# nanoporetech/pomfret

Hardware: AMD Instinct MI355X
Metric: aligned reads/sec (methphase kernel) (higher is better)
Workload: dtype u32/f32

## Files before the change

### pomfret_amd/csrc/pf_kernels.hip

```cpp
#include <hip/hip_runtime.h>
#include <stdint.h>
#include "pf_device.h"

#define DEV static __device__ __forceinline__

#ifdef PF_K3_PROFILE
DEV unsigned long long k3_stamp_now() {
    unsigned long long t;
    __builtin_amdgcn_sched_barrier(0);
    asm volatile("s_memtime %0\n\ts_waitcnt lgkmcnt(0)" : "=s"(t) :: "memory");
    __builtin_amdgcn_sched_barrier(0);
    return t;
}
#define K3_STAMP(i) do { const unsigned long long t_ = k3_stamp_now(); \
    prof_acc[i] += t_ - prof_last; prof_last = t_; } while (0)
DEV unsigned long long k3_realtime() {
    unsigned long long t;
    asm volatile("s_memrealtime %0\n\ts_waitcnt lgkmcnt(0)" : "=s"(t) :: "memory");
    return t;
}
#define K3_COUNT(i, v) do { prof_acc[i] += (v); } while (0)
#define K12_STAMP(i) do { if (threadIdx.x == 0) { const unsigned long long t_ = k3_stamp_now(); \
    d.prof[64ull * d.W + (uint64_t)w * 16 + (i)] = t_ - k12_t0; k12_t0 = t_; } } while (0)
#define K2_STAMP(i) do { if (k2acc) { const unsigned long long t_ = k3_stamp_now(); \
    k2acc[i] += t_ - k2acc[9]; k2acc[9] = t_; } } while (0)
#else
#define K12_STAMP(i) do { } while (0)
#define K2_STAMP(i) do { } while (0)
#define K3_STAMP(i) do { } while (0)
#define K3_COUNT(i, v) do { } while (0)
#endif

#ifdef PF_ASM_MARK
#define K3_MARK(s) asm volatile("; MARK " s)
#else
#define K3_MARK(s) do { } while (0)
#endif

DEV uint32_t uni(uint32_t x) { return (uint32_t)__builtin_amdgcn_readfirstlane((int)x); }
DEV int uni_i(int x) { return __builtin_amdgcn_readfirstlane(x); }

DEV uint64_t lanemask_lt(uint32_t lane) { return lane ? (~0ull >> (64 - lane)) : 0ull; }

DEV void wave_sync() {
    __builtin_amdgcn_fence(__ATOMIC_RELEASE, "wavefront");
    __builtin_amdgcn_wave_barrier();
    __builtin_amdgcn_fence(__ATOMIC_ACQUIRE, "wavefront");
}

DEV void wave_sync_mem() {
    __builtin_amdgcn_fence(__ATOMIC_RELEASE, "workgroup");
    __builtin_amdgcn_wave_barrier();
    __builtin_amdgcn_fence(__ATOMIC_ACQUIRE, "workgroup");
}

DEV uint32_t wave_incl_scan(uint32_t x, uint32_t lane) {
#pragma unroll
    for (int o = 1; o < 64; o <<= 1) {
        uint32_t y = __shfl_up(x, o, 64);
        if (lane >= (uint32_t)o) x += y;
    }
    return x;
}

DEV uint32_t wave_max_u32(uint32_t x) {
#pragma unroll
    for (int o = 32; o > 0; o >>= 1) { uint32_t y = __shfl_xor(x, o, 64); x = y > x ? y : x; }
    return x;
}

DEV uint32_t dpp_max_step(uint32_t x, const int ctrl_sel) {
    uint32_t y;
    switch (ctrl_sel) {
    case 0: y = (uint32_t)__builtin_amdgcn_update_dpp(0, (int)x, 0xB1, 0xF, 0xF, false); break;
    case 1: y = (uint32_t)__builtin_amdgcn_update_dpp(0, (int)x, 0x4E, 0xF, 0xF, false); break;
    case 2: y = (uint32_t)__builtin_amdgcn_update_dpp(0, (int)x, 0x141, 0xF, 0xF, false); break;
    default: y = (uint32_t)__builtin_amdgcn_update_dpp(0, (int)x, 0x140, 0xF, 0xF, false); break;
    }
    return y > x ? y : x;
}
DEV uint32_t wave_max_dpp(uint32_t x) {
    x = dpp_max_step(x, 0);
    x = dpp_max_step(x, 1);
    x = dpp_max_step(x, 2);
    x = dpp_max_step(x, 3);
    const uint32_t a = (uint32_t)__builtin_amdgcn_readlane((int)x, 0), b = (uint32_t)__builtin_amdgcn_readlane((int)x, 16);
    const uint32_t c = (uint32_t)__builtin_amdgcn_readlane((int)x, 32), e = (uint32_t)__builtin_amdgcn_readlane((int)x, 48);
    const uint32_t ab = a > b ? a : b, ce = c > e ? c : e;
    return ab > ce ? ab : ce;
}
DEV uint32_t wave_shl1(uint32_t x) {
    return (uint32_t)__builtin_amdgcn_update_dpp(0, (int)x, 0x130, 0xF, 0xF, false);
}
DEV float div_u16_y(float fa, float fb, float y) {
    const float q0 = fa * y;
    const float r = __builtin_fmaf(-q0, fb, fa);
    return __builtin_fmaf(r, y, q0);
}
DEV float div_u16(uint32_t a, uint32_t b) {
    const float fb = (float)b;
    return div_u16_y((float)a, fb, __builtin_amdgcn_rcpf(fb));
}
DEV float4 site_rec(uint32_t v) {
    const uint32_t h0 = v & 0xffffu, h1 = v >> 16;
    const float f0 = (float)(h0 ? h0 : 1u), f1 = (float)(h1 ? h1 : 1u);
    return make_float4(f0, f1, h0 ? __builtin_amdgcn_rcpf(f0) : 0.f, h1 ? __builtin_amdgcn_rcpf(f1) : 0.f);
}

DEV uint32_t dpp_shr_add(uint32_t x, const int ctrl) {
    uint32_t y;
    switch (ctrl) {
    case 1: y = (uint32_t)__builtin_amdgcn_update_dpp(0, (int)x, 0x111, 0xF, 0xF, true); break;
    case 2: y = (uint32_t)__builtin_amdgcn_update_dpp(0, (int)x, 0x112, 0xF, 0xF, true); break;
// ... 1225 lines not shown
            const uint32_t r = r0 + i;
            d.mmr_off[2 * r] = kcarry + 2ull * e1;
            d.mmr_off[2 * r + 1] = kcarry + 2ull * e1 + bound;
            d.big_off[r] = bigb ? bcarry + e2 : ~0ull;
        }
        kcarry += 2ull * t1;
        bcarry += t2;
    }

    K12_STAMP(5);
    const uint32_t arr_b = (uint32_t)((14ull * S + 15) & ~15ull);
    if (tid == 0) sh_misc[5] = NW;
    __syncthreads();

    if (staged && R >= d.k12c_minr && S <= d.k12c_smax) {
        for (uint32_t c = tid; c * PF_K12C_READS < R; c += NT) {
            const uint32_t k = atomicAdd(d.k12c_ctr, 1u);
            d.k12c_list[2ull * k] = w;
            d.k12c_list[2ull * k + 1] = c * PF_K12C_READS;
        }
    } else if (staged) {
        uint8_t *wb = reinterpret_cast<uint8_t *>(tile) + arr_b + wid * (uint64_t)PF_K12_WB * PF_K12_CAPW;
#ifdef PF_K3_PROFILE
        unsigned long long k2a[10] = {0, 0, 0, 0, 0, 0, 0, 0, 0, __builtin_amdgcn_s_memtime()};
        unsigned long long *k2acc = wid == 0 ? k2a : nullptr;
#else
        unsigned long long *k2acc = nullptr;
#endif
        k12_methmers(d, r0, 0, R, wid, NW, lane, S, sp, st1, q1s, l0s, l1s, wb, k2acc, &sh_misc[5]);
#ifdef PF_K3_PROFILE
        if (tid == 0) {
            for (int j = 0; j < 7; j++) d.prof[64ull * d.W + (uint64_t)w * 16 + 8 + j] = k2a[j];
            d.prof[64ull * d.W + (uint64_t)w * 16 + 7] = k2a[7];
            d.prof[64ull * d.W + (uint64_t)w * 16 + 15] = k2a[8];
        }
#endif
    } else {
        for (uint32_t i = tid; i < R; i += NT) d.fb_list[atomicAdd(d.fb_ctr, 1u)] = r0 + i;
    }
    __syncthreads();
    K12_STAMP(6);
}

__global__ __launch_bounds__(PF_K12C_WAVES * 64) __attribute__((amdgpu_waves_per_eu(4, 4))) void pf_k12_chunks(pf_dev_batch d) {
    extern __shared__ __attribute__((aligned(16))) uint8_t smem[];
    __shared__ uint32_t s_item, s_rctr;
    const uint32_t tid = threadIdx.x, lane = tid & 63u, wid = uni(tid >> 6);
    const uint32_t n = *d.k12c_ctr;
    for (;;) {
        if (tid == 0) s_item = atomicAdd(d.k12c_next, 1u);
        __syncthreads();
        const uint32_t it = s_item;
        if (it >= n) break;
        const uint32_t w = d.k12c_list[2ull * it], c0 = d.k12c_list[2ull * it + 1];
        if (tid == 0) s_rctr = c0 + PF_K12C_WAVES;
        const uint32_t r0 = d.win_read_off[w], R = d.win_read_off[w + 1] - r0;
        const uint32_t S = d.win_S[w];
        const uint64_t sb = d.win_site_off[w];
        uint32_t *sp = reinterpret_cast<uint32_t *>(smem), *st1 = sp + S, *q1s = sp + 2 * S;
        uint8_t *l0s = reinterpret_cast<uint8_t *>(sp + 3 * S), *l1s = l0s + S;
        for (uint32_t p = tid; p < S; p += PF_K12C_WAVES * 64) {
            sp[p] = d.site_pos[sb + p];
            st1[p] = d.st1_pos[sb + p];
            q1s[p] = d.site_q1[sb + p];
            l0s[p] = d.len0[sb + p];
            l1s[p] = d.len1[sb + p];
        }
        __syncthreads();
        const uint32_t arr_b = (uint32_t)((14ull * S + 15) & ~15ull);
        uint8_t *wb = smem + arr_b + wid * (uint64_t)PF_K12_WB * PF_K12_CAPW;
        const uint32_t c1 = min(R, c0 + PF_K12C_READS);
        k12_methmers(d, r0, c0, c1, wid, PF_K12C_WAVES, lane, S, sp, st1, q1s, l0s, l1s, wb, nullptr,
                     &s_rctr);
        __syncthreads();
    }
}

struct K3Ctl {
    uint32_t S, R, ntot, nc, L, done, failed, inserted, winner, tag;
    int32_t i_last;
    uint32_t min_i, max_i, fail, summ, nstrict, mxlen, cmax;
    uint32_t path, need, cacheb;
    unsigned long long t_run;
    uint32_t ins_n, ins_st, ins_mo, ins_tg;
    unsigned long long scr;
    int32_t tab[4];
};

struct K3Cand {
    uint32_t read[PF_MAX_NCAND];
    uint32_t pos[PF_MAX_NCAND];
    uint32_t site0[PF_MAX_NCAND];
    uint32_t len[PF_MAX_NCAND];
    uint32_t kofs[PF_MAX_NCAND];
    unsigned long long key[PF_MAX_NCAND];
    uint8_t tag[PF_MAX_NCAND];
};

template <int NTH>
struct K3CandSlimT {
    uint32_t read[NTH];
    uint32_t pos[128];
    unsigned long long key[256];
};
using K3CandSlim = K3CandSlimT<PF_K3S_THREADS>;

DEV uint64_t align16(uint64_t x) { return (x + 15) & ~15ull; }

template <int NT, typename K, typename F>
DEV void k3_each_key(const pf_dev_batch &d, uint32_t r0, uint32_t R, uint32_t dir, K &&keep, F &&f) {
    constexpr uint32_t B = 8, NW = NT / 64;
    const uint32_t lane = threadIdx.x & 63, wid = threadIdx.x >> 6;
    for (uint32_t i0 = wid * B; i0 < R; i0 += NW * B) {
        uint32_t n[B], st[B], key[B];
        uint64_t off[B];
#pragma unroll
        for (uint32_t u = 0; u < B; u++) {
            const uint32_t i = i0 + u;
            const bool ok = i < R && keep(i);
            const uint64_t g = 2ull * (r0 + (ok ? i : 0u)) + dir;
            n[u] = ok ? d.mmr_n[g] : 0u;
            st[u] = d.mmr_start[g];
            off[u] = d.mmr_off[g];
        }
#pragma unroll
        for (uint32_t u = 0; u < B; u++) key[u] = lane < n[u] ? d.keys[off[u] + lane] : 0u;
#pragma unroll
        for (uint32_t u = 0; u < B; u++)
            if (lane < n[u]) f(i0 + u, lane, st[u] + lane, off[u] + lane, key[u]);
#pragma unroll
        for (uint32_t u = 0; u < B; u++)
            for (uint32_t t = 64 + lane; t < n[u]; t += 64) f(i0 + u, t, st[u] + t, off[u] + t, d.keys[off[u] + t]);
    }
}

template <int NT = PF_K3_THREADS>
DEV void k3_dict(const pf_dev_batch &d, uint32_t r0, uint32_t R, uint32_t S, uint32_t dir,
                 uint64_t *masks, uint32_t *base, uint32_t *sh_scan, K3Ctl &ctl) {
    const uint32_t tid = threadIdx.x;
    const uint32_t MW = (uint32_t)d.mw;
    for (uint32_t j = tid; j < S * MW; j += NT) masks[j] = 0;
    __syncthreads();
    k3_each_key<NT>(d, r0, R, dir, [](uint32_t) { return true; },
                    [&](uint32_t, uint32_t, uint32_t site, uint64_t, uint32_t key) {
                        if (site < S && key < 64u * MW)
                            atomicOr((unsigned long long *)&masks[(uint64_t)site * MW + (key >> 6)], 1ull << (key & 63));
                    });
    __syncthreads();
    uint32_t carry = 0;
    for (uint32_t p0 = 0; p0 < S; p0 += NT) {
        const uint32_t p = p0 + tid;
        uint32_t c = 0;
        if (p < S)
            for (uint32_t m = 0; m < MW; m++) c += (uint32_t)__popcll(masks[(uint64_t)p * MW + m]);
        uint32_t tot;
        const uint32_t ex = block_excl_scan<NT>(c, sh_scan, &tot);
        if (p < S) base[p] = carry + ex;
        carry += tot;
    }
    if (tid == 0) ctl.ntot = carry;
    __syncthreads();
}

template <int NT = PF_K3_THREADS>
DEV void k3_dict_rewrite(const pf_dev_batch &d, uint32_t r0, uint32_t R, uint32_t S, uint32_t dir,
                         const uint64_t *masks, const uint32_t *base) {
    const uint32_t MW = (uint32_t)d.mw;
    k3_each_key<NT>(d, r0, R, dir, [](uint32_t) { return true; },
                    [&](uint32_t, uint32_t, uint32_t site, uint64_t koff, uint32_t key) {
                        uint32_t slot = PF_NONE;
                        if (site < S && key < 64u * MW) {
                            const uint64_t *row = masks + (uint64_t)site * MW;
                            const uint32_t wi = key >> 6, b = key & 63;
                            slot = base[site];
                            for (uint32_t m = 0; m < wi; m++) slot += (uint32_t)__popcll(row[m]);
                            slot += (uint32_t)__popcll(row[wi] & ((1ull << b) - 1ull));
                        }
                        d.keys[koff] = slot;
                    });
    __syncthreads();
}

DEV uint32_t kd_hash(uint32_t key) {
    const uint32_t h = key * 0x9E3779B1u;
    return h ^ (h >> 15);
}
DEV void kd_sync() {
    __builtin_amdgcn_fence(__ATOMIC_RELEASE, "agent");
    __syncthreads();
    __builtin_amdgcn_fence(__ATOMIC_ACQUIRE, "agent");
}

__global__ __launch_bounds__(PF_K3_THREADS) void pf_k3_kdict(pf_dev_batch d) {
    constexpr uint32_t NT = PF_K3_THREADS, NW = NT / 64;
    __shared__ uint32_t sh_scan[NW + 1];
    __shared__ unsigned long long s_o;
    __shared__ uint32_t s_fail;
    const uint32_t prob = blockIdx.x, w = prob >> 1, dir = prob & 1;
    const uint32_t tid = threadIdx.x, lane = tid & 63u, wid = tid >> 6;
    const uint32_t S = d.win_S[w];
    if (S == 0) {
        if (tid == 0) d.k3_ntot[prob] = 0;
        return;
    }
    const uint32_t R = d.win_nreads[w], r0 = d.win_read_off[w];
    auto alloc = [&](uint64_t bytes) -> bool {
        if (tid == 0) {
            const unsigned long long o = atomicAdd(d.scr_ctr, (unsigned long long)bytes);
            s_fail = o + bytes > d.scr_cap;
            if (s_fail) atomicOr(d.status, PF_ST_SCR_OVF);
            s_o = o;
        }
        __syncthreads();
        return s_fail == 0;
    };
    if (!alloc(align16(12ull * (S + 1)))) { if (tid == 0) d.k3_ntot[prob] = PF_NONE; return; }
    uint32_t *cap = reinterpret_cast<uint32_t *>(d.scr + s_o), *toff = cap + (S + 1), *base = toff + (S + 1);
    for (uint32_t j = tid; j <= S; j += NT) cap[j] = 0;
    kd_sync();
    for (uint32_t i = tid; i < R; i += NT) {
        const uint64_t g = 2ull * (r0 + i) + dir;
        const uint32_t n = d.mmr_n[g], st = d.mmr_start[g];
        if (n && st < S) {
            atomicAdd(&cap[st], 1u);
            atomicAdd(&cap[st + n < S ? st + n : S], 0xFFFFFFFFu);
        }
    }
    kd_sync();
    const uint32_t per = (S + NT - 1) / NT, j0 = min(tid * per, S), j1 = min(j0 + per, S);
    uint32_t part = 0, tot = 0;
    for (uint32_t j = j0; j < j1; j++) part += cap[j];
// ... 590 lines not shown
template <bool SLDS, int NT = PF_K3_THREADS, bool C8 = false>
DEV void k3_init(const pf_dev_batch &d, uint32_t w, uint32_t dir, uint32_t r0, uint32_t S, uint32_t R,
                 const K3Mem &m, K3Ctl &ctl, uint32_t *sh_scan, K3Stats &stx) {
    const uint32_t tid = threadIdx.x, lane = tid & 63, wid = uni(tid >> 6);
    const uint32_t ntot = uni(ctl.ntot);
    const int cov_rt = d.win_par[w * 4 + 1];
    const uint32_t s = d.win_start[w], e = d.win_end[w];
    const uint32_t nwords = (R + 63) >> 6;
    const uint64_t sb = d.win_site_off[w];
    const uint64_t kbase = d.mmr_off[2ull * r0];
    const uint32_t *kb = d.keys + kbase;
    uint32_t sum_mmr = 0, mx_mmr = 0;
    for (uint32_t j = tid; j < (C8 ? (ntot + 1) / 2 : ntot); j += NT) m.cnt[j] = 0;
    for (uint32_t j = tid; j < S; j += NT) m.sum[j] = 0;
    for (uint32_t i = tid; i < R; i += NT) {
        const uint32_t r = r0 + i;
        const uint32_t st = d.read_start[r], en = d.read_end[r];
        uint32_t f = 0;
        if (st <= s) {
            f |= FLG_LEFT;
            if (en > s) f |= FLG_LEFT_STRICT;
        } else if (en >= e) {
            f |= FLG_RIGHT;
            if (st < e) f |= FLG_RIGHT_STRICT;
        }
        m.flg[i] = (uint8_t)f;
        m.hp[i] = d.read_hp[r];
        m.aux[i] = 0;
        if (dir) m.ord[i] = (uint16_t)d.rev_ord[r];
        const uint64_t g = 2ull * r + dir;
        const uint32_t n_ = d.mmr_n[g], st_ = d.mmr_start[g];
        if (!m.mn) {
        } else if (m.m16) {
            static_cast<uint16_t *>(m.mn)[i] = (uint16_t)n_;
            static_cast<uint16_t *>(m.mst)[i] = (uint16_t)st_;
        } else {
            static_cast<uint32_t *>(m.mn)[i] = n_;
            static_cast<uint32_t *>(m.mst)[i] = st_;
        }
        sum_mmr += n_;
        mx_mmr = n_ > mx_mmr ? n_ : mx_mmr;
    }
    if (tid == 0) {
        const uint32_t *a = d.site_pos + sb;
        if (dir == 0) {
            ctl.min_i = 0;
            ctl.max_i = (uint32_t)ub_u32(a, 0, S, s);
        } else {
            ctl.max_i = S - 1;
            ctl.min_i = (uint32_t)((int)ub_u32(a, 0, S, e) - 1);
        }
        ctl.i_last = dir == 0 ? 0 : (int)R - 1;
        ctl.failed = 0;
        ctl.done = 0;
        ctl.tab[0] = 0;
    }
    __syncthreads();
    if (SLDS) {
        uint32_t carry = 0;
        for (uint32_t i0 = 0; i0 < R; i0 += NT) {
            const uint32_t i = i0 + tid;
            const uint32_t v = i < R ? k3_mn(m, i) : 0;
            uint32_t tot;
            const uint32_t ex = block_excl_scan<NT>(v, sh_scan, &tot);
            if (i < R) m.mo[i] = carry + ex;
            carry += tot;
        }
        __syncthreads();
        for (uint32_t i = wid; i < R; i += (NT / 64)) {
            const uint32_t g = 2 * (r0 + i) + dir;
            const uint32_t *src = kb + (d.mmr_off[g] - kbase);
            uint16_t *dst = m.sl16 + m.mo[i];
            const uint32_t n = k3_mn(m, i);
            for (uint32_t t = lane; t < n; t += 64) {
                const uint32_t v = src[t];
                dst[t] = v == PF_NONE ? (uint16_t)0xFFFFu : (uint16_t)v;
            }
        }
    } else if (m.mo) {
        for (uint32_t i = tid; i < R; i += NT)
            m.mo[i] = (uint32_t)(d.mmr_off[2ull * (r0 + i) + dir] - kbase);
    }
    __syncthreads();
    const uint32_t refbit = dir == 0 ? FLG_LEFT : FLG_RIGHT;
    uint32_t ref_ins = 0;
    auto seed = [&](uint32_t i, uint32_t site, uint32_t slot) {
        const uint32_t hp = m.hp[i];
        if (site < S && slot != PF_NONE) {
            if (C8) atomicAdd(&m.cnt[slot >> 1], (hp ? 0x100u : 1u) << ((slot & 1u) * 16u));
            else atomicAdd(&m.cnt[slot], hp ? 0x10000u : 1u);
            atomicAdd(&m.sum[site], hp ? 0x10000u : 1u);
        }
    };
    auto is_ref = [&](uint32_t i) { return (m.flg[i] & refbit) && m.hp[i] <= 1; };
    if (SLDS) {
        for (uint32_t i = wid; i < R; i += (NT / 64)) {
            if (!is_ref(i)) continue;
            const uint32_t n = k3_mn(m, i), st = k3_mst(m, i), mo = m.mo[i];
            ref_ins += n;
            for (uint32_t t = lane; t < n; t += 64) seed(i, st + t, k3_slot<SLDS>(m, mo + t));
        }
    } else {
        k3_each_key<NT>(d, r0, R, dir, is_ref, [&](uint32_t i, uint32_t t, uint32_t site, uint64_t, uint32_t slot) {
            if (t == 0) ref_ins += d.mmr_n[2ull * (r0 + i) + dir];
            seed(i, site, slot);
        });
        ref_ins = (uint32_t)__builtin_amdgcn_readfirstlane((int)ref_ins);
    }
    if (lane == 0 && ref_ins) atomicAdd((uint32_t *)&ctl.tab[0], ref_ins);
    if (sum_mmr) atomicAdd(&ctl.summ, sum_mmr);
    if (mx_mmr) atomicMax(&ctl.mxlen, mx_mmr);
    __syncthreads();
    if (wid == 0) k3_range_update(m.sum, S, cov_rt, ctl, lane);
    for (uint32_t i = tid; i < R; i += NT) {
        if (m.flg[i] & refbit) {
            const uint32_t t = i | ((uint32_t)m.hp[i] >> 2);
            if (t < R) atomicMax(&m.aux[t], i + 1);
        }
    }
    __syncthreads();
    for (uint32_t i = tid; i < R; i += NT) {
        const uint32_t lw = m.aux[i];
        m.hp[i] = lw ? (uint8_t)(d.read_hp[r0 + lw - 1] & 3) : (uint8_t)2;
    }
    __syncthreads();
    for (uint32_t j = wid; j < nwords; j += (NT / 64)) {
        const uint32_t p = j * 64 + lane;
        bool u = false;
        if (p < R) {
            const uint32_t rd = dir ? m.ord[p] : p;
            const uint32_t h = m.hp[rd];
            u = h != 0 && h != 1;
        }
        const uint64_t b = __ballot(u);
        if (lane == 0) m.untag[j] = b;
    }
    stx.inserts = ctl.tab[0];
    __syncthreads();
}

DEV void k3_finish(const pf_dev_batch &d, uint32_t w, uint32_t dir, uint32_t r0, uint32_t S, uint32_t R,
                   const K3Mem &m, const K3Ctl &ctl, const K3Stats &stx) {
    const uint32_t lane = threadIdx.x & 63;
    int tab0 = 0, tab1 = 0, tab2 = 0, tab3 = 0;
    uint32_t nstrict = 0;
    const uint32_t strict = dir == 0 ? FLG_RIGHT_STRICT : FLG_LEFT_STRICT;
    for (uint32_t i = lane; i < R; i += 64) {
        if (m.flg[i] & strict) {
            nstrict++;
            const uint32_t ref = d.read_hp[r0 + i], q = m.hp[i];
            if (ref <= 1 && q <= 1) {
                const uint32_t k = ref * 2 + q;
                tab0 += k == 0; tab1 += k == 1; tab2 += k == 2; tab3 += k == 3;
            }
        }
        if (dir == 0) d.hp_fwd[r0 + i] = m.hp[i];
    }
    uint32_t tsum[5] = {(uint32_t)tab0, (uint32_t)tab1, (uint32_t)tab2, (uint32_t)tab3, nstrict};
#pragma unroll
    for (int k = 0; k < 5; k++) {
        uint32_t tot = 0;
        for (int bb = 0; bb < 16; bb++) tot += (uint32_t)__popcll(__ballot((tsum[k] >> bb) & 1)) << bb;
        tsum[k] = tot;
    }
    if (lane < 4) d.table[((uint64_t)w * 2 + dir) * 4 + lane] = (int32_t)tsum[lane];
    if (lane == 0) {
        unsigned long long *sp = d.stats + ((uint64_t)w * 2 + dir) * PF_NSTAT;
        sp[0] = stx.lookups; sp[1] = stx.inserts; sp[3] = stx.scanned;
        sp[2] = stx.iters | ((unsigned long long)ctl.path << 56);
        sp[4] = ctl.summ; sp[5] = tsum[4]; sp[6] = R; sp[7] = S;
    }
}


DEV void k3_range_regs(const K3Mem &m, uint32_t S, int cov_rt, uint32_t lane, uint32_t &umin, uint32_t &umax) {
    auto cov_ok = [&](int ii) -> bool {
        const uint32_t v = m.sum[ii];
        return (int)((v & 0xffffu) + (v >> 16)) >= cov_rt;
    };
    const int m0 = (int)umin, M0 = (int)umax;
    const bool left = lane < 32;
    const int i = left ? m0 - (int)lane : M0 + (int)(lane - 32);
    bool cvg = false;
    if (left ? (m0 >= 0 && i >= 0) : (M0 >= 0 && i < (int)S)) cvg = cov_ok(i);
    const uint64_t b = __ballot(cvg);
    const uint32_t bl = (uint32_t)b, br = (uint32_t)(b >> 32);
    int cl = bl == ~0u ? 32 : __ffs(~bl) - 1;
    int cr = br == ~0u ? 32 : __ffs(~br) - 1;
    if (cl == 32) {
        for (;;) {
            const int ii = m0 - cl - (int)lane;
            const uint64_t b2 = __ballot(ii >= 0 && cov_ok(ii));
            if (b2 == ~0ull) { cl += 64; continue; }
            cl += __ffsll((unsigned long long)~b2) - 1;
            break;
        }
    }
    if (cr == 32) {
        for (;;) {
            const int ii = M0 + cr + (int)lane;
            const uint64_t b2 = __ballot(ii < (int)S && cov_ok(ii));
            if (b2 == ~0ull) { cr += 64; continue; }
            cr += __ffsll((unsigned long long)~b2) - 1;
            break;
        }
    }
    if (m0 >= 0 && cl > 0) umin = (uint32_t)(m0 - cl + 1);
    if (M0 >= 0 && cr > 0) umax = (uint32_t)(M0 + cr - 1);
}

template <bool SLDS, int NT = PF_K3_THREADS, bool C8 = false, bool CACHE = false, typename CD = K3Cand>
DEV void k3_greedy_slim(const pf_dev_batch &d, uint32_t w, uint32_t dir, uint32_t r0, uint32_t S, uint32_t R,
                        const K3Mem &m, K3Ctl &ctl, CD &cd, uint32_t *sh_scan, uint32_t *qb, uint32_t CL = 0) {
    const uint32_t tid = threadIdx.x, lane = tid & 63, wid = uni(tid >> 6);
    const int cov_rt = d.win_par[w * 4 + 1];
    const uint32_t NC = (uint32_t)d.win_par[w * 4 + 2];
    const uint32_t nwords = (R + 63) >> 6;
    K3Stats stx = {0, 0, 0, 0};
#ifdef PF_K3_PROFILE
    unsigned long long prof_acc[32] = {0};
    unsigned long long prof_last = k3_stamp_now();
// ... 152 lines not shown
                float s0 = 0.f, s1 = 0.f;
                if (lane < nc) k3_fold_direct<SLDS, C8>(m, c_lo, c_kofs, c_len, s0, s1);
                const float diff = s0 > s1 ? s0 - s1 : s1 - s0;
                const bool elig = lane < nc && !(diff < 3.f && (l0 < 3 || l1 < 3));
                const uint32_t hkey = elig ? __float_as_uint(diff) + 1u : 0u;
                const uint32_t hmax = wave_max_dpp(hkey);
                if (hmax == 0) pick = 2;
                else {
                    pick = 1;
                    cw = 63u - (uint32_t)__clzll((long long)__ballot(hkey == hmax));
                    tg = rdl(s0 > s1 ? 0u : 1u, cw);
                }
            }
        }
        par ^= 1;
        K3_STAMP(19);
        if (pick == 2) {
            if (++failed > 10) break;
            il += dir == 0 ? (int)NC : -(int)NC;
            need_collect = true;
            have_win = false;
            __syncthreads();
            continue;
        }
        const uint32_t rd = rdl(c_rd, cw), n = rdl(c_n, cw), st = rdl(c_st, cw);
        const uint32_t mo = CACHE ? rdl(c_cs, cw) * CL : rdl(c_mo, cw);
        const uint32_t pw = rdl(c_pos, cw);
        stx.inserts += n;
        if (wid == 0 && lane == 0) {
            m.hp[rd] = (uint8_t)tg;
            m.untag[pw >> 6] &= ~(1ull << (pw & 63));
        }
        failed = 0;
        if (CACHE) fmask |= 1ull << (mo / CL);
        {
            const uint32_t a0 = wave_shl1(c_pos), a1 = wave_shl1(c_rd), a2 = wave_shl1(c_n), a3 = wave_shl1(c_st);
            const uint32_t a4 = CACHE ? 0u : wave_shl1(c_mo);
            const uint32_t a5 = CACHE ? wave_shl1(c_cs) : 0u;
            if (lane >= cw) { c_pos = a0; c_rd = a1; c_n = a2; c_st = a3; c_mo = a4; c_cs = a5; }
        }
        {
            const uint32_t te = st + n;
            auto hit = [&](uint32_t a) { return a != 0xFFFFFFFFu && a >= st && a < te; };
            rng_walk = !have_win || hit(umin) || hit(umin - 1u) || hit(umax) || hit(umax + 1u);
        }
        uint32_t ncn = nc - 1;
        if (qn >= 0) {
            if (lane == ncn) { c_pos = (uint32_t)qn; c_rd = q_rd1; c_n = q_n1; c_st = q_st1; c_mo = q_mo1; c_cs = s_sp; }
            if (CACHE) fmask &= ~(1ull << s_sp);
            ncn++;
        }
        nc = ncn;
        if (nc == 0) need_collect = true;
        K3_STAMP(20);
        if (folded) __syncthreads();
        k3_insert_all<SLDS, NT, C8>(m, S, n, st, mo, tg);
        if (CACHE && qn >= 0) {
            uint16_t *dst = m.sl16 + s_sp * CL;
            if (tid < q_n1) dst[tid] = pf0 == PF_NONE ? (uint16_t)0xFFFFu : (uint16_t)pf0;
            if (tid + NT < q_n1) dst[tid + NT] = pf1 == PF_NONE ? (uint16_t)0xFFFFu : (uint16_t)pf1;
        }
        have_win = true;
        K3_STAMP(21);
        __syncthreads();
        K3_STAMP(8);
    }
    {
        uint32_t tot = 0;
#pragma unroll
        for (int bb = 0; bb < 32; bb++) tot += (uint32_t)__popcll(__ballot((lsum >> bb) & 1)) << bb;
        stx.lookups += tot;
    }
    if (wid != 0) return;
    k3_finish(d, w, dir, r0, S, R, m, ctl, stx);
#ifdef PF_K3_PROFILE
    if (lane == 0) {
        unsigned long long *pp = d.prof + ((uint64_t)w * 2 + dir) * 32;
        prof_acc[29] = ctl.path;
        prof_acc[25] = k3_realtime();
        prof_acc[26] = ctl.t_run;
        prof_acc[30] = ctl.ntot;
        prof_acc[31] = ctl.need;
        prof_acc[27] = ctl.cacheb;
        for (int i = 0; i < 32; i++) pp[i] = prof_acc[i];
    }
#endif
}

template <bool SLDS, bool FULL>
DEV void k3_greedy_body(const pf_dev_batch &d, uint32_t w, uint32_t dir, uint32_t r0, uint32_t S,
                        uint32_t R, const K3Mem &m, K3Ctl &ctl, K3Cand &cd, uint32_t *sh_scan) {
    const uint32_t tid = threadIdx.x, lane = tid & 63, wid = uni(tid >> 6);
    const int cov_rt = d.win_par[w * 4 + 1];
    const uint32_t NC = (uint32_t)d.win_par[w * 4 + 2];
    const uint32_t nwords = (R + 63) >> 6;
    K3Stats stx = {0, 0, 0, 0};
#ifdef PF_K3_PROFILE
    unsigned long long prof_acc[32] = {0};
    unsigned long long prof_last = k3_stamp_now();
#endif

    k3_init<SLDS>(d, w, dir, r0, S, R, m, ctl, sh_scan, stx);

    K3_STAMP(0);
    const uint32_t rec_cap = PF_K3_WAVES * m.rcw;
    if (!FULL || NC <= 64) {
    int il = uni_i(ctl.i_last);
    uint32_t failed = 0;
    uint32_t umin = uni(ctl.min_i), umax = uni(ctl.max_i);
    uint32_t nc = 0;
    uint32_t c_pos = 0, c_rd = 0, c_n = 0, c_st = 0, c_mo = 0;
    uint32_t c_lo = 0, c_len = 0, c_kofs = 0;
    uint32_t q_pos = 0, q_rd = 0, q_nn = 0, q_st = 0, q_mo = 0;
    uint32_t q_cnt = 0, q_head = 0;
    bool q_more = false;
    int q_cont = 0;
    uint32_t *qbuf = cd.read;
    uint32_t lsum = 0;
    const bool exact_path = !FULL || (uni(ctl.mxlen) < 8192u && d.k3_mode != 2u);
    K3_COUNT(15, exact_path ? 1 : 0);
    bool need_collect = true, stop = false;
    int qn = -1;
    uint32_t q_rd1 = 0, q_n1 = 0, q_st1 = 0, q_mo1 = 0;
    uint32_t p_n = 0, p_st = 0, p_mo = 0, p_tg = 0;
    uint32_t *lcp = reinterpret_cast<uint32_t *>(cd.key);
    double *accd = reinterpret_cast<double *>(cd.key + 128);
    K3_STAMP(1);
    for (;;) {
    if (wid == 0) {
        K3_STAMP(28);
        if (!stop && need_collect) {
            bool done = false;
            for (;;) {
                if (dir == 0 ? il >= (int)R : il <= 0) { done = true; break; }
                K3_COUNT(25, 1);
                q_cnt = k3_qbuild(m, nwords, dir == 0 ? il - 1 : il + 1, dir, lane, qbuf,
                                  q_pos, q_rd, q_nn, q_st, q_mo, q_more, q_cont);
                const uint32_t take = q_cnt < NC ? q_cnt : NC;
                c_pos = q_pos; c_rd = q_rd; c_n = q_nn; c_st = q_st; c_mo = q_mo;
                q_head = take;
                uint32_t found = take;
                while (found < NC && q_more) {
                    K3_COUNT(26, 1);
                    q_cnt = k3_qbuild(m, nwords, q_cont, dir, lane, qbuf, q_pos, q_rd, q_nn, q_st, q_mo,
                                      q_more, q_cont);
                    q_head = 0;
                    while (found < NC && q_head < q_cnt) {
                        const uint32_t a0 = rdl(q_pos, q_head), a1 = rdl(q_rd, q_head), a2 = rdl(q_nn, q_head);
                        const uint32_t a3 = rdl(q_st, q_head), a4 = rdl(q_mo, q_head);
                        if (lane == found) { c_pos = a0; c_rd = a1; c_n = a2; c_st = a3; c_mo = a4; }
                        found++;
                        q_head++;
                    }
                }
                if (found == 0) {
                    stx.scanned += dir == 0 ? (uint32_t)((int)R - il) : (uint32_t)(il + 1);
                    if (++failed > 10) { done = true; break; }
                    il += dir == 0 ? (int)NC : -(int)NC;
                    continue;
                }
                nc = found;
                break;
            }
            if (done) stop = true;
        }
        K3_STAMP(16);
// ... 440 lines not shown
                    k3_scanned(ctl, cd, R, dir, NC, stx);
                }
            } else {
                k3_cand_fields(m, ncn, dir, lane, ctl, cd, stx);
                k3_scanned(ctl, cd, R, dir, NC, stx);
            }
        }
        K3_STAMP(7);
    }
    }

    k3_finish(d, w, dir, r0, S, R, m, ctl, stx);
    if (lane == 0) {
#ifdef PF_K3_PROFILE
        unsigned long long *pp = d.prof + ((uint64_t)w * 2 + dir) * 32;
        for (int i = 0; i < 32; i++) pp[i] = prof_acc[i];
#endif
    }
}

DEV void k3_defer(const pf_dev_batch &d, uint32_t prob) {
    if (threadIdx.x == 0) d.k3_fb_list[atomicAdd(d.k3_fb_ctr, 1u)] = prob;
}

DEV bool k3_scr_alloc(const pf_dev_batch &d, K3Ctl &ctl, uint64_t bytes, bool reuse) {
    if (reuse) __syncthreads();
    if (threadIdx.x == 0) {
        ctl.fail = 0;
        if (bytes) {
            const unsigned long long o = atomicAdd(d.scr_ctr, (unsigned long long)align16(bytes));
            if (o + bytes > d.scr_cap) { ctl.fail = 1; atomicOr(d.status, PF_ST_SCR_OVF); }
            ctl.scr = o;
        }
    }
    __syncthreads();
    return !uni(ctl.fail);
}

template <bool FULL, int NT = PF_K3_THREADS, typename CD = K3Cand>
DEV void k3_run(const pf_dev_batch &d, uint32_t prob, uint8_t *smem, K3Ctl &ctl, CD &cd, uint32_t *sh_scan,
                const uint32_t lds, uint32_t *qb = nullptr) {
    static_assert(sizeof(cd.read) / sizeof(cd.read[0]) >= (size_t)NT, "cd.read holds 64 entries per wave");
    const uint32_t tid = threadIdx.x;
    const uint32_t w = prob >> 1, dir = prob & 1;
    const uint32_t S = d.win_S[w];
    if (S == 0) {
        if (tid < 4) d.table[((uint64_t)w * 2 + dir) * 4 + tid] = 0;
        if (tid < PF_NSTAT) d.stats[((uint64_t)w * 2 + dir) * PF_NSTAT + tid] = 0;
        return;
    }
    const uint32_t R = d.win_nreads[w];
    const uint32_t r0 = d.win_read_off[w];
    const uint32_t MW = (uint32_t)d.mw;
    const uint64_t kbase = d.mmr_off[2ull * r0];
#ifdef PF_K3_PROFILE
    if (tid == 0) ctl.t_run = k3_realtime();
#endif

    const bool kd = d.kdict != 0u;
    const uint64_t need1 = kd ? 0ull : align16(8ull * S * MW) + 4ull * S;
    const bool p1_lds = need1 <= lds;
    const bool slim_ok = p1_lds && d.win_par[w * 4 + 2] <= 64 && S < 8192u && d.k3_mode == 0u;
    if (!FULL && !slim_ok) {
        k3_defer(d, prob);
        return;
    }
    if (tid == 0) {
        ctl.summ = 0;
        ctl.nstrict = 0;
        ctl.mxlen = 0;
    }
    if (!k3_scr_alloc(d, ctl, p1_lds ? 0ull : need1, false)) return;
    uint64_t *masks;
    uint32_t *mbase;
    if (!FULL || p1_lds) {
        masks = reinterpret_cast<uint64_t *>(smem);
        mbase = reinterpret_cast<uint32_t *>(smem + align16(8ull * S * MW));
    } else {
        uint8_t *g = d.scr + ctl.scr;
        masks = reinterpret_cast<uint64_t *>(g);
        mbase = reinterpret_cast<uint32_t *>(g + align16(8ull * S * MW));
    }
    if (!kd) k3_dict<NT>(d, r0, R, S, dir, masks, mbase, sh_scan, ctl);
    const uint32_t ntot = kd ? uni(d.k3_ntot[prob]) : uni(ctl.ntot);
    if (kd && ntot == PF_NONE) return;
    if (kd && tid == 0) ctl.ntot = ntot;
    uint32_t summ = 0, lmx = 0;
    for (uint32_t i = tid; i < R; i += NT) {
        const uint32_t n_ = d.mmr_n[2ull * (r0 + i) + dir];
        summ += n_;
        lmx = n_ > lmx ? n_ : lmx;
    }
    if (lmx) atomicMax(&ctl.mxlen, lmx);
    uint32_t summ_tot;
    block_excl_scan<NT>(summ, sh_scan, &summ_tot);

    const bool slots_ok = ntot < 0xFFFFu;
    bool c8 = false;
    if (slim_ok && (!FULL || p1_lds) && need1 + align16(4ull * (S + 1)) <= lds) {
        uint32_t *cov = reinterpret_cast<uint32_t *>(smem + need1);
        for (uint32_t j = tid; j <= S; j += NT) cov[j] = 0;
        if (tid == 0) ctl.cmax = 0;
        __syncthreads();
        for (uint32_t i = tid; i < R; i += NT) {
            const uint64_t g = 2ull * (r0 + i) + dir;
            const uint32_t n = d.mmr_n[g], st = d.mmr_start[g];
            if (n && st < S) {
                atomicAdd(&cov[st], 1u);
                atomicAdd(&cov[st + n < S ? st + n : S], 0xFFFFFFFFu);
            }
        }
        __syncthreads();
        const uint32_t per = (S + NT) / NT;
        const uint32_t j0 = tid * per, j1 = min(j0 + per, S + 1);
        uint32_t part = 0;
        for (uint32_t j = j0; j < j1; j++) part += cov[j];
        uint32_t tot;
        uint32_t run = block_excl_scan<NT>(part, sh_scan, &tot), mx = 0;
        for (uint32_t j = j0; j < j1; j++) { run += cov[j]; mx = run > mx ? run : mx; }
        if (mx) atomicMax(&ctl.cmax, mx);
        __syncthreads();
        c8 = uni(ctl.cmax) < 256u;
    }
    auto lay = [&](K3Place p, uint32_t rcw, bool c8_) { return k3_layout(S, ntot, R, dir, summ_tot, p, rcw, c8_); };
    const K3Layout l_lists = lay(K3Place::Lists, 0, c8), l_hbm = lay(K3Place::Hbm, 0, c8);
    const K3Layout l_cache = lay(K3Place::Cache, 0, c8), l_gcnt = lay(K3Place::CacheGcnt, 0, c8);
    const uint32_t CL = (uni(ctl.mxlen) + 1u) & ~1u;
    const uint32_t NCc = (uint32_t)d.win_par[w * 4 + 2];
    const bool cache_ok = slim_ok && slots_ok && NCc <= 63u && CL > 0 && CL <= 2u * NT && (d.k3_cache & 1u) != 0u;
    const bool lists_ok = slots_ok && d.k3_cache < 2u;
    const uint64_t cache_b = 2ull * (NCc + 1) * CL;
    const uint64_t slim_c = align16(l_cache.need) + cache_b, slim_g = align16(l_gcnt.need) + cache_b;
    const uint32_t slim = !slim_ok ? 0u : (lists_ok && l_lists.need <= lds) ? 1u : (cache_ok && slim_c <= lds) ? 2u
                        : l_hbm.need <= lds ? 3u : 0u;
    const bool gcnt = !FULL && cache_ok && c8 && slim_g <= lds && (!slim || d.k3_gcnt != 0u);
    const uint32_t path = gcnt ? 6u : slim ? slim : FULL ? 4u : 0u;
    if (!path) {
        k3_defer(d, prob);
        return;
    }
    if (path == 6u && !k3_scr_alloc(d, ctl, align16(2ull * ntot), true)) return;
    if (!kd) k3_dict_rewrite<NT>(d, r0, R, S, dir, masks, mbase);
    if (tid == 0) {
        ctl.path = path;
#ifdef PF_K3_PROFILE
        ctl.need = (uint32_t)(cache_ok ? slim_c : path == 1 ? l_lists.need : l_hbm.need);
        ctl.cacheb = (uint32_t)cache_b;
#endif
    }
    K3Mem m;
    uint32_t *qq = qb ? qb : cd.read;
    switch (path) {
    case 1:
        k3_mem(d, r0, dir, kbase, S, smem, l_lists, m);
        if (c8) k3_greedy_slim<true, NT, true, false, CD>(d, w, dir, r0, S, R, m, ctl, cd, sh_scan, qq);
        else k3_greedy_slim<true, NT, false, false, CD>(d, w, dir, r0, S, R, m, ctl, cd, sh_scan, qq);
        return;
    case 2:
        k3_mem(d, r0, dir, kbase, S, smem, l_cache, m);
        if (c8) k3_greedy_slim<true, NT, true, true, CD>(d, w, dir, r0, S, R, m, ctl, cd, sh_scan, qq, CL);
        else k3_greedy_slim<true, NT, false, true, CD>(d, w, dir, r0, S, R, m, ctl, cd, sh_scan, qq, CL);
        return;
    case 3:
        k3_mem(d, r0, dir, kbase, S, smem, l_hbm, m);
        if (c8) k3_greedy_slim<false, NT, true, false, CD>(d, w, dir, r0, S, R, m, ctl, cd, sh_scan, qq);
        else k3_greedy_slim<false, NT, false, false, CD>(d, w, dir, r0, S, R, m, ctl, cd, sh_scan, qq);
        return;
    case 6:
        if constexpr (!FULL) {
            k3_mem(d, r0, dir, kbase, S, smem, l_gcnt, m, d.scr + ctl.scr);
            k3_greedy_slim<true, NT, true, true, CD>(d, w, dir, r0, S, R, m, ctl, cd, sh_scan, qq, CL);
        }
        return;
    }
    if constexpr (FULL) {
        const uint32_t rcw_min = 256, rcw_max = 1024;
        auto grown = [&](const K3Layout &l) {
            const uint32_t rcw = (uint32_t)((lds - l.tail) / (12ull * PF_K3_WAVES));
            return lay(l.place, rcw > rcw_max ? rcw_max : rcw, false);
        };
        const K3Layout b_lists = lay(K3Place::Lists, rcw_min, false), b_hbm = lay(K3Place::Hbm, rcw_min, false);
        if (slots_ok && b_lists.need <= lds) {
            k3_mem(d, r0, dir, kbase, S, smem, grown(b_lists), m);
            k3_greedy_body<true, true>(d, w, dir, r0, S, R, m, ctl, cd, sh_scan);
        } else if (b_hbm.need <= lds) {
            k3_mem(d, r0, dir, kbase, S, smem, grown(b_hbm), m);
            k3_greedy_body<false, true>(d, w, dir, r0, S, R, m, ctl, cd, sh_scan);
        } else {
            if (!k3_scr_alloc(d, ctl, align16(b_hbm.need), true)) return;
            k3_mem(d, r0, dir, kbase, S, d.scr + ctl.scr, b_hbm, m);
            k3_greedy_body<false, true>(d, w, dir, r0, S, R, m, ctl, cd, sh_scan);
        }
    }
}

__global__ __launch_bounds__(PF_K3S_THREADS) __attribute__((amdgpu_waves_per_eu(4))) void pf_k3_greedy(pf_dev_batch d) {
    extern __shared__ __attribute__((aligned(16))) uint8_t smem[];
    __shared__ K3Ctl ctl;
    __shared__ K3CandSlim cd;
    __shared__ uint32_t sh_scan[PF_K3S_THREADS / 64 + 1];
    __shared__ uint32_t s_rank;
    static_assert(PF_K3S_THREADS <= PF_MAX_NCAND, "cd.read holds the per-wave queue scratch");
    for (;;) {
        if (threadIdx.x == 0) s_rank = atomicAdd(d.k3_next, 1u);
        __syncthreads();
        const uint32_t rank = uni(s_rank);
        if (rank >= d.k3_n) break;
        k3_run<false, PF_K3S_THREADS>(d, d.k3_order[rank], smem, ctl, cd, sh_scan, d.lds_bytes);
        __syncthreads();
    }
}

__global__ __launch_bounds__(PF_K3H_THREADS) __attribute__((amdgpu_waves_per_eu(4))) void pf_k3_heavy(pf_dev_batch d) {
    extern __shared__ __attribute__((aligned(16))) uint8_t smem[];
    __shared__ K3Ctl ctl;
    __shared__ K3CandSlimT<PF_K3H_THREADS> cd;
    __shared__ uint32_t sh_scan[PF_K3H_THREADS / 64 + 1];
    k3_run<false, PF_K3H_THREADS>(d, d.k3_order[blockIdx.x], smem, ctl, cd, sh_scan, d.lds_heavy);
}

__global__ __launch_bounds__(PF_K3_THREADS) void pf_k3_fallback(pf_dev_batch d) {
    extern __shared__ __attribute__((aligned(16))) uint8_t smem[];
    __shared__ K3Ctl ctl;
    __shared__ K3Cand cd;
    __shared__ uint32_t sh_scan[PF_K3_WAVES + 1];
// ... 851 lines not shown
```

Measured before the change: 61.96 million.

## Pack read key segments across lanes with prefetched metadata in k3_each_key

Replaces the per-wave eight-reads-per-round key traversal with a lane-packed scheme. Each lane owns one read's metadata, a wave prefix scan splits reads into 64-key segments, and segments are distributed densely so short reads no longer leave lanes idle. The next chunk's metadata is prefetched, and key loads are batched G*8 deep to overlap memory latency. It also adds profiling stamps that compile away by default. In exchange it spends readlane, ballot and scan work on every segment and increases register pressure.

```diff
diff --git a/pomfret_amd/csrc/pf_kernels.hip b/pomfret_amd/csrc/pf_kernels.hip
--- a/pomfret_amd/csrc/pf_kernels.hip
+++ b/pomfret_amd/csrc/pf_kernels.hip
@@ -20,6 +20,7 @@
     return t;
 }
 #define K3_COUNT(i, v) do { prof_acc[i] += (v); } while (0)
+#define K3_SETUP_STAMP(ctl, i) do { if (threadIdx.x == 0) (ctl).t_st[i] = k3_realtime(); } while (0)
 #define K12_STAMP(i) do { if (threadIdx.x == 0) { const unsigned long long t_ = k3_stamp_now(); \
     d.prof[64ull * d.W + (uint64_t)w * 16 + (i)] = t_ - k12_t0; k12_t0 = t_; } } while (0)
 #define K2_STAMP(i) do { if (k2acc) { const unsigned long long t_ = k3_stamp_now(); \
@@ -29,6 +30,7 @@
 #define K2_STAMP(i) do { } while (0)
 #define K3_STAMP(i) do { } while (0)
 #define K3_COUNT(i, v) do { } while (0)
+#define K3_SETUP_STAMP(ctl, i) do { } while (0)
 #endif
 
 #ifdef PF_ASM_MARK
@@ -1420,6 +1422,9 @@
     uint32_t min_i, max_i, fail, summ, nstrict, mxlen, cmax;
     uint32_t path, need, cacheb;
     unsigned long long t_run;
+#ifdef PF_K3_PROFILE
+    unsigned long long t_st[7];
+#endif
     uint32_t ins_n, ins_st, ins_mo, ins_tg;
     unsigned long long scr;
     int32_t tab[4];
@@ -1445,8 +1450,75 @@
 
 DEV uint64_t align16(uint64_t x) { return (x + 15) & ~15ull; }
 
+#ifndef PF_K3_PIPE
+#define PF_K3_PIPE 1
+#endif
+template <int NT, uint32_t G, typename K, typename F>
+DEV void k3_each_key_lanes(const pf_dev_batch &d, uint32_t r0, uint32_t R, uint32_t dir, K &&keep, F &&f) {
+    constexpr uint32_t B = 8, RS = NT / 64 * B, CH = 8 * RS;
+    static_assert(G == 1 || G == 2 || G == 4 || G == 8, "a chunk's eight rounds in whole batches");
+    uint32_t lane = threadIdx.x & 63;
+    asm volatile("" : "+v"(lane));
+    const uint32_t wid = uni(threadIdx.x >> 6);
+    const uint64_t kbase = d.mmr_off[2ull * r0];
+    const uint32_t *kb = d.keys + kbase;
+    const uint32_t il = (lane >> 3) * RS + wid * B + (lane & 7);
+    auto fields = [&](uint32_t c0, uint32_t &n, uint32_t &st, uint32_t &ko) {
+        const uint32_t i = c0 + il;
+        n = st = ko = 0u;
+        if (i < R && keep(i)) {
+            const uint64_t g = 2ull * (r0 + i) + dir;
+            n = d.mmr_n[g];
+            st = d.mmr_start[g];
+            ko = (uint32_t)(d.mmr_off[g] - kbase);
+        }
+    };
+    auto bcast = [](uint32_t v, uint32_t l) { return (uint32_t)__builtin_amdgcn_readlane((int)v, (int)l); };
+    constexpr uint32_t SB = G * B;
+    uint32_t nv, stv, kov;
+    fields(0, nv, stv, kov);
+    for (uint32_t c0 = 0; c0 < R; c0 += CH) {
+        uint32_t nn, stn, kon;
+        fields(c0 + CH, nn, stn, kon);
+        const uint32_t incl = wave_incl_scan_dpp((nv + 63u) >> 6);
+        const uint32_t nseg = bcast(incl, 63);
+        auto seg_of = [&](uint32_t g, uint32_t &l, uint32_t &t0, uint32_t &n) {
+            const uint32_t r = (uint32_t)__popcll(__ballot(incl <= g));
+            l = r < 64u ? r : 63u;
+            const uint32_t before = l ? bcast(incl, l - 1u) : 0u;
+            t0 = g < nseg ? (g - before) << 6 : PF_NONE;
+            n = g < nseg ? bcast(nv, l) : 0u;
+        };
+        for (uint32_t g0 = 0; g0 < nseg; g0 += SB) {
+            uint32_t key[SB];
+#pragma unroll
+            for (uint32_t j = 0; j < SB; j++) {
+                uint32_t l, t0, n;
+                seg_of(g0 + j, l, t0, n);
+                const uint32_t ko = bcast(kov, l);
+                key[j] = t0 != PF_NONE && t0 + lane < n ? kb[ko + t0 + lane] : 0u;
+            }
+#pragma unroll 1
+            for (uint32_t j0 = 0; j0 < SB && g0 + j0 < nseg; j0 += B) {
+#pragma unroll
+                for (uint32_t u = 0; u < B; u++) {
+                    uint32_t l, t0, n;
+                    seg_of(g0 + j0 + u, l, t0, n);
+                    const uint32_t st = bcast(stv, l), ko = bcast(kov, l);
+                    const uint32_t i = c0 + (l >> 3) * RS + wid * B + (l & 7u), t = t0 + lane;
+                    if (t0 != PF_NONE && t < n) f(i, t, st + t, kbase + ko + t, key[u]);
+                }
+#pragma unroll
+                for (uint32_t j = 0; j + B < SB; j++) key[j] = key[j + B];
+            }
+        }
+        nv = nn;
+        stv = stn;
+        kov = kon;
+    }
+}
 template <int NT, typename K, typename F>
-DEV void k3_each_key(const pf_dev_batch &d, uint32_t r0, uint32_t R, uint32_t dir, K &&keep, F &&f) {
+DEV void k3_each_key_rounds(const pf_dev_batch &d, uint32_t r0, uint32_t R, uint32_t dir, K &&keep, F &&f) {
     constexpr uint32_t B = 8, NW = NT / 64;
     const uint32_t lane = threadIdx.x & 63, wid = threadIdx.x >> 6;
     for (uint32_t i0 = wid * B; i0 < R; i0 += NW * B) {
@@ -1470,6 +1542,14 @@
         for (uint32_t u = 0; u < B; u++)
             for (uint32_t t = 64 + lane; t < n[u]; t += 64) f(i0 + u, t, st[u] + t, off[u] + t, d.keys[off[u] + t]);
     }
+}
+template <int NT, uint32_t G = 4, typename K, typename F>
+DEV void k3_each_key(const pf_dev_batch &d, uint32_t r0, uint32_t R, uint32_t dir, K &&keep, F &&f) {
+#if PF_K3_PIPE
+    k3_each_key_lanes<NT, G>(d, r0, R, dir, keep, f);
+#else
+    k3_each_key_rounds<NT>(d, r0, R, dir, keep, f);
+#endif
 }
 
 template <int NT = PF_K3_THREADS>
@@ -1485,6 +1565,7 @@
                             atomicOr((unsigned long long *)&masks[(uint64_t)site * MW + (key >> 6)], 1ull << (key & 63));
                     });
     __syncthreads();
+    K3_SETUP_STAMP(ctl, 0);
     uint32_t carry = 0;
     for (uint32_t p0 = 0; p0 < S; p0 += NT) {
         const uint32_t p = p0 + tid;
@@ -2241,6 +2322,7 @@
             m.mo[i] = (uint32_t)(d.mmr_off[2ull * (r0 + i) + dir] - kbase);
     }
     __syncthreads();
+    K3_SETUP_STAMP(ctl, 4);
     const uint32_t refbit = dir == 0 ? FLG_LEFT : FLG_RIGHT;
     uint32_t ref_ins = 0;
     auto seed = [&](uint32_t i, uint32_t site, uint32_t slot) {
@@ -2260,7 +2342,7 @@
             for (uint32_t t = lane; t < n; t += 64) seed(i, st + t, k3_slot<SLDS>(m, mo + t));
         }
     } else {
-        k3_each_key<NT>(d, r0, R, dir, is_ref, [&](uint32_t i, uint32_t t, uint32_t site, uint64_t, uint32_t slot) {
+        k3_each_key<NT, 2>(d, r0, R, dir, is_ref, [&](uint32_t i, uint32_t t, uint32_t site, uint64_t, uint32_t slot) {
             if (t == 0) ref_ins += d.mmr_n[2ull * (r0 + i) + dir];
             seed(i, site, slot);
         });
@@ -2270,6 +2352,7 @@
     if (sum_mmr) atomicAdd(&ctl.summ, sum_mmr);
     if (mx_mmr) atomicMax(&ctl.mxlen, mx_mmr);
     __syncthreads();
+    K3_SETUP_STAMP(ctl, 5);
     if (wid == 0) k3_range_update(m.sum, S, cov_rt, ctl, lane);
     for (uint32_t i = tid; i < R; i += NT) {
         if (m.flg[i] & refbit) {
@@ -2296,6 +2379,7 @@
     }
     stx.inserts = ctl.tab[0];
     __syncthreads();
+    K3_SETUP_STAMP(ctl, 6);
 }
 
 DEV void k3_finish(const pf_dev_batch &d, uint32_t w, uint32_t dir, uint32_t r0, uint32_t S, uint32_t R,
@@ -2614,6 +2698,10 @@
         prof_acc[30] = ctl.ntot;
         prof_acc[31] = ctl.need;
         prof_acc[27] = ctl.cacheb;
+        {
+            const int sl[7] = {15, 16, 17, 18, 22, 23, 28};
+            for (int i = 0; i < 7; i++) prof_acc[sl[i]] = ctl.t_st[i];
+        }
         for (int i = 0; i < 32; i++) pp[i] = prof_acc[i];
     }
 #endif
@@ -3220,6 +3308,8 @@
         mbase = reinterpret_cast<uint32_t *>(g + align16(8ull * S * MW));
     }
     if (!kd) k3_dict<NT>(d, r0, R, S, dir, masks, mbase, sh_scan, ctl);
+    else K3_SETUP_STAMP(ctl, 0);
+    K3_SETUP_STAMP(ctl, 1);
     const uint32_t ntot = kd ? uni(d.k3_ntot[prob]) : uni(ctl.ntot);
     if (kd && ntot == PF_NONE) return;
     if (kd && tid == 0) ctl.ntot = ntot;
@@ -3278,7 +3368,9 @@
         return;
     }
     if (path == 6u && !k3_scr_alloc(d, ctl, align16(2ull * ntot), true)) return;
+    K3_SETUP_STAMP(ctl, 2);
     if (!kd) k3_dict_rewrite<NT>(d, r0, R, S, dir, masks, mbase);
+    K3_SETUP_STAMP(ctl, 3);
     if (tid == 0) {
         ctl.path = path;
 #ifdef PF_K3_PROFILE
```

Result: no change. 62.05 million (median of 4 runs) (+0.1%).
